# ssteinberg/wave_tracer

Measured on AMD Instinct MI355X. Metric: Msamples/sec (whole node), cornell-box 1440^2 wave-mode, higher is better.
Workload: dtype f32

## Files before the change

wave_tracer_amd/csrc/kernels_path.hip:

```cpp
#include "wtgpu_kernels.h"

namespace wtk {

__global__ void __launch_bounds__(kBlock) k_path_generate(launch_args_t a) {
    const uint32_t i = blockIdx.x * kBlock + threadIdx.x;
    if (i == 0) {
        uint32_t* ctl = a.st.ctl;
        ctl[CTL_COUNT0] = a.nb;
        ctl[CTL_COUNT1] = 0;
        ctl[CTL_BACK0] = ctl[CTL_BACK1] = 0;
        ctl[CTL_UTD_COUNT0] = ctl[CTL_UTD_COUNT1] = ctl[CTL_FSDQ_COUNT0] = ctl[CTL_FSDQ_COUNT1] = ctl[CTL_FSDQ_HEAD] = ctl[CTL_NEEQ_COUNT] = ctl[CTL_NEEQ_HEAD] = 0;
        ctl[CTL_HEAD_TRACE] = ctl[CTL_HEAD_INTERACT] = ctl[CTL_HEAVY_COUNT] = ctl[CTL_HEAVY_HEAD] = ctl[CTL_FSD_COUNTER] = ctl[CTL_ROUNDS] = 0;
        ctl[CTL_TPOL_COUNT0] = ctl[CTL_TPOL_COUNT1] = ctl[CTL_TPOL_HEAD] = ctl[CTL_TCONE_COUNT0] = ctl[CTL_TCONE_COUNT1] = ctl[CTL_TCONE_HEAD] = 0;
        ctl[CTL_INTB_COUNT] = ctl[CTL_INTB_HEAD] = ctl[CTL_GATHER_COUNT] = ctl[CTL_GATHER_HEAD] = ctl[CTL_INTC_COUNT] = ctl[CTL_INTC_HEAD] = 0;
        ctl[CTL_FTASK_COUNT] = ctl[CTL_FTASK_HEAD] = ctl[CTL_FSPLIT_HEAD] = ctl[CTL_EPOOL_COUNT] = ctl[CTL_FSD_ECOUNTER] = 0;
        ctl[CTL_INTD_COUNT] = ctl[CTL_INTD_HEAD] = 0;
    }
    if (i >= a.nb) return;
    const uint64_t j = a.j0 + i;
    const uint32_t pix = (uint32_t)(j % a.npix);
    const uint64_t s = a.sample_begin + j / a.npix;
    const uint64_t sample_id = ((uint64_t)pix << 32) | (s & 0xFFFFFFFFull);
    path_walk_t pw;
    path_generate(a.sc, a.seed, sample_id, pix % a.sc.sensor.width, pix / a.sc.sensor.width, pw);
    soa_store(a.st.walks, a.st.walk_words, i, pw);
}

#ifdef WTGPU_FSD_WATCH
// ... 241 lines not shown
```

wave_tracer_amd/csrc/kernels_trace.hip:

```cpp
#include "wtgpu_kernels.h"

namespace wtk {

}
#include "kernels_trace_refill.h"
namespace wtk {

__global__ void __launch_bounds__(kBlock, WTGPU_LB_TRACE) k_trace_refill(launch_args_t a, int in, int first_round, uint32_t round) { trace_refill_body(a, in, first_round, round); }

#ifndef WTGPU_SM_EXACT_MIN
#define WTGPU_SM_EXACT_MIN 24
#endif
#ifndef WTGPU_SM_SPLIT_NODE
#define WTGPU_SM_SPLIT_NODE 0
#endif
#ifndef WTGPU_SM_BOTH
#define WTGPU_SM_BOTH 0
#endif
enum : int { PH_IDLE = 0, PH_NODE = 1, PH_TRI = 2, PH_EXACT = 3, PH_SERVE = 4, PH_POLICY = 5, PH_RAYDONE = 6 };
#ifdef WTGPU_SM_PROF
#define SP_DECL() unsigned long long sp_t[8] = {0, 0, 0, 0, 0, 0, 0, 0}, sp_l[8] = {0, 0, 0, 0, 0, 0, 0, 0}, sp_n[8] = {0, 0, 0, 0, 0, 0, 0, 0}; long long sp_c = 0
#define SP_BEGIN() sp_c = clock64()
#define SP_END(i, mask) do { const long long d_ = clock64() - sp_c; sp_t[i] += (unsigned long long)d_; sp_l[i] += (unsigned long long)d_ * (unsigned long long)__popcll(mask); sp_n[i] += 1; } while (0)
#else
// ... 300 lines not shown
    for (;;) {
        const int need = aw_next(sc, env, rt, stack, aw, q, r);
        if (need != AW_TEST) return need == AW_QUERY;
        aw_test_done(aw, cone_attempt_too_short_by(sc, env, aw.cand, aw.sr, aw.min_df_prog));
    }
}
#ifndef WTGPU_LB_STAGE
#define WTGPU_LB_STAGE 3
#endif
__global__ void __launch_bounds__(kBlock, WTGPU_LB_STAGE) k_tr_axis(launch_args_t a, int in, int first_round, uint32_t round) {
    __shared__ stack_entry_t lds[kLdsStack * kBlock];
    uint32_t* ctl = a.st.ctl;
    const uint32_t n = queue_count(ctl, in);
    if (blockIdx.x == 0 && threadIdx.x == 0) {
        trace_round_begin(ctl, in, round, n);
        ctl[CTL_TCONE_HEAD] = 0;
        ctl[CTL_TPOL_COUNT1] = 0;
    }
    bdpt_counters_t ctr;
    memset(&ctr, 0, sizeof(ctr));
    stack_entry_t spill[kSpillStack];
    stack_ref_t stack;
    lds_stack(lds, spill, stack);
    const bool rt = a.sc.sensor.ray_trace_only || a.sc.opts.force_ray_tracing;
    const int lane = threadIdx.x & 63;
    uint32_t* stage = trace_stage_words(a);
    uint32_t* coneq = trace_cone_queue(a);
    for (;;) {
        const uint32_t base = wave_grab(ctl + CTL_HEAD_TRACE);
        if (base >= n) break;
        const uint32_t qi = base + (uint32_t)lane;
        bool fin = false, query = false;
        uint32_t w = 0;
        trav_result_t r;
        if (qi < n) {
            w = queue_walk(a, ctl, in, qi, first_round);
            const walk_trace_in_t wk = walk_load_trace_in(a.st.walks, a.st.walk_words, w);
            trace_stage_t ts;
            ts.env = walk_trace_envelope(a.sc, wk);
            ray_hit_t ah;
            const bool axis_hit = ads_intersect_ray(a.sc, ts.env.o, ts.env.d, range_t{0.f, WT_INF}, stack, ah);
            aw_begin(ts.aw, wavenum_to_wavelen_m(wk.k), WT_INF, axis_hit, ah, a.cone_budget, true, !(a.collect_list & 1u) || (a.collect_list & 2u), a.lane_cache ? wk.prev_offset_tuid : kInvalid);
            ts.aw.use_cache = a.lane_cache;
            query = tr_policy_run(a.sc, ts.env, rt, stack, ts.aw, r);
            fin = !query;
            if (query) soa_store(stage, kStageWords, w, ts);
        }
        wave_append(coneq, ctl + CTL_TCONE_COUNT0, query, w);
        tr_finish(a, ctl, ctr, fin, w, r);
    }
    if (a.count_stats) flush_counters(a.st.counters, ctr);
}
#ifndef WTGPU_CONE_REFILL_MIN
#define WTGPU_CONE_REFILL_MIN 16
#endif
#ifndef WTGPU_CONE_DEFER
#define WTGPU_CONE_DEFER 0
#endif
__global__ void __launch_bounds__(kBlock, WTGPU_LB_STAGE) k_tr_cone(launch_args_t a, uint32_t it) {
    __shared__ stack_entry_t lds[kLdsStack * kBlock];
#if WTGPU_CONE_DEFER
    __shared__ float lds_tri[12 * kBlock];
    float* my_tri = lds_tri + threadIdx.x;
    bool wait = false;
#endif
    uint32_t* ctl = a.st.ctl;
    const uint32_t n = ctl[CTL_TCONE_COUNT0 + (it & 1u)];
    if (blockIdx.x == 0 && threadIdx.x == 0) {
        ctl[CTL_TPOL_HEAD] = 0;
        ctl[CTL_TCONE_COUNT0 + ((it + 1u) & 1u)] = 0;
    }
    bdpt_counters_t ctr;
    memset(&ctr, 0, sizeof(ctr));
    stack_entry_t spill[kSpillStack];
    stack_ref_t stack;
    lds_stack(lds, spill, stack);
    const lane_nodes_t ns = lane_nodes(a.sc);
    const int lane = threadIdx.x & 63;
    const unsigned long long below = (1ull << lane) - 1ull;
    uint32_t* stage = trace_stage_words(a);
    const uint32_t* coneq = trace_cone_queue(a);
    uint32_t* polq = trace_pol_queue(a);
    uint32_t* pol_count = ctl + CTL_TPOL_COUNT0 + ((it + 1u) & 1u);
    int st = 0;
    uint32_t w = 0;
    cone_t env;
    cone_query_t q;
    memset(&env, 0, sizeof(env));
    memset(&q, 0, sizeof(q));
    bool exhausted = false;
    SP_DECL();
    for (;;) {
        uint32_t* slot = a.st.tris + (size_t)w * kTriListWords;
        const uint_list_t tris{slot, 1u, (a.collect_list & 1u) ? kMaxConeTris : 0u, reinterpret_cast<float*>(slot + kMaxConeTris)};
        bool fin = false, again = false;
        trav_result_t r;
        SP_BEGIN();
        const unsigned long long sp_m0 = __ballot(st == 2);
        (void)sp_m0;
        if (st == 2) {
            cq_end(env, tris, q);
            axis_walk_t aw;
            soa_load(stage + offsetof(trace_stage_t, aw) / 4, kStageWords, w, aw);
            fin = aw_query_done(a.sc, env, aw, q.rec, r);
            again = !fin;
            if (again) {
                stage[(size_t)w * kStageWords + (offsetof(trace_stage_t, aw) + offsetof(axis_walk_t, seg)) / 4] = aw.seg;
                stage[(size_t)w * kStageWords + (offsetof(trace_stage_t, aw) + offsetof(axis_walk_t, short_tuid)) / 4] = aw.short_tuid;
            }
            st = 0;
        }
        wave_append(polq, pol_count, again, w);
        tr_finish(a, ctl, ctr, fin, w, r);
        SP_END(0, sp_m0);
        {
            const unsigned long long im = __ballot(st == 0);
            const int n_run = __popcll(__ballot(st == 1));
            if (!exhausted && im && (__popcll(im) >= WTGPU_CONE_REFILL_MIN || n_run == 0)) {
                uint32_t base = 0;
                if (lane == 0) base = atomicAdd(ctl + CTL_TCONE_HEAD, (uint32_t)__popcll(im));
                base = (uint32_t)__shfl((int)base, 0, 64);
                if (base + (uint32_t)__popcll(im) >= n) exhausted = true;
                const uint32_t qi = base + (uint32_t)__popcll(im & below);
                SP_BEGIN();
                const unsigned long long sp_m1 = __ballot(st == 0 && qi < n);
                (void)sp_m1;
                if (st == 0 && qi < n) {
                    w = coneq[qi];
                    soa_load(stage, kStageWords, w, env);
                    const size_t o = (size_t)w * kStageWords + offsetof(trace_stage_t, aw) / 4;
                    const range_t sr{__uint_as_float(stage[o + offsetof(axis_walk_t, sr) / 4]), __uint_as_float(stage[o + offsetof(axis_walk_t, sr) / 4 + 1])};
                    const float min_df_prog = __uint_as_float(stage[o + offsetof(axis_walk_t, min_df_prog) / 4]);
                    cq_begin(a.sc, env, sr, kMajorAxisToZScale, stack, a.cone_budget, min_df_prog, q);
                    st = cq_running(q) ? 1 : 2;
                }
                SP_END(1, sp_m1);
            }
        }
        const int running = __popcll(__ballot(st == 1));
        if (running == 0) {
            if (__ballot(st == 2)) continue;
            if (exhausted) break;
            continue;
// ... 91 lines not shown
#endif
    }
    if (a.count_stats) flush_counters(a.st.counters, ctr);
#ifdef WTGPU_SM_PROF
    if (lane == 0)
        for (int i = 0; i < 8; ++i) {
            atomicAdd(a.st.counters + kNumCounters + 32 + i, sp_t[i]);
            atomicAdd(a.st.counters + kNumCounters + 40 + i, sp_l[i]);
            atomicAdd(a.st.counters + kNumCounters + 48 + i, sp_n[i]);
        }
#endif
}
__global__ void __launch_bounds__(kBlock, WTGPU_LB_STAGE) k_tr_policy(launch_args_t a, uint32_t it) {
    __shared__ stack_entry_t lds[kBlock];
    uint32_t* ctl = a.st.ctl;
    const uint32_t n = ctl[CTL_TPOL_COUNT0 + (it & 1u)];
    if (blockIdx.x == 0 && threadIdx.x == 0) {
        ctl[CTL_TCONE_HEAD] = 0;
        ctl[CTL_TPOL_COUNT0 + ((it + 1u) & 1u)] = 0;
    }
    bdpt_counters_t ctr;
    memset(&ctr, 0, sizeof(ctr));
    const stack_ref_t stack = make_stack_ref(lds + threadIdx.x, kBlock, 1, 1, nullptr);
    const bool rt = a.sc.sensor.ray_trace_only || a.sc.opts.force_ray_tracing;
    const int lane = threadIdx.x & 63;
    uint32_t* stage = trace_stage_words(a);
    const uint32_t* polq = trace_pol_queue(a);
    uint32_t* coneq = trace_cone_queue(a);
    for (;;) {
        const uint32_t base = wave_grab(ctl + CTL_TPOL_HEAD);
        if (base >= n) break;
        const uint32_t qi = base + (uint32_t)lane;
        bool fin = false, query = false;
        uint32_t w = 0;
        trav_result_t r;
        if (qi < n) {
            w = polq[qi];
            trace_stage_t ts;
            soa_load(stage, kStageWords, w, ts);
            query = tr_policy_run(a.sc, ts.env, rt, stack, ts.aw, r);
            fin = !query;
            if (query) soa_store(stage + offsetof(trace_stage_t, aw) / 4, kStageWords, w, ts.aw);
        }
        wave_append(coneq, ctl + CTL_TCONE_COUNT0 + (it & 1u), query, w);
        tr_finish(a, ctl, ctr, fin, w, r);
    }
    if (a.count_stats) flush_counters(a.st.counters, ctr);
}
__global__ void __launch_bounds__(kBlock, WTGPU_LB_TRACE) k_tr_tail(launch_args_t a, uint32_t it) {
    __shared__ stack_entry_t lds[kLdsStack * kBlock];
    uint32_t* ctl = a.st.ctl;
    const uint32_t n = ctl[CTL_TPOL_COUNT0 + (it & 1u)];
    if (blockIdx.x == 0 && threadIdx.x == 0) ctl[CTL_TCONE_COUNT0] = ctl[CTL_TCONE_COUNT1] = 0;
    bdpt_counters_t ctr;
    memset(&ctr, 0, sizeof(ctr));
    stack_entry_t spill[kSpillStack];
    stack_ref_t stack;
    lds_stack(lds, spill, stack);
    const lane_nodes_t ns = lane_nodes(a.sc);
    const bool rt = a.sc.sensor.ray_trace_only || a.sc.opts.force_ray_tracing;
    const int lane = threadIdx.x & 63;
    uint32_t* stage = trace_stage_words(a);
    const uint32_t* polq = trace_pol_queue(a);
    for (;;) {
        const uint32_t base = wave_grab(ctl + CTL_TPOL_HEAD);
        if (base >= n) break;
        const uint32_t qi = base + (uint32_t)lane;
        const bool have = qi < n;
        uint32_t w = 0;
        trav_result_t r;
        if (have) {
            w = polq[qi];
            trace_stage_t ts;
            soa_load(stage, kStageWords, w, ts);
            uint32_t* slot = a.st.tris + (size_t)w * kTriListWords;
            const uint_list_t tris{slot, 1u, (a.collect_list & 1u) ? kMaxConeTris : 0u, reinterpret_cast<float*>(slot + kMaxConeTris)};
            cone_query_t q;
            for (;;) {
                const int need = aw_next(a.sc, ts.env, rt, stack, ts.aw, q, r);
                if (need == AW_FINAL) break;
                if (need == AW_TEST) {
                    aw_test_done(ts.aw, cone_attempt_too_short_by(a.sc, ts.env, ts.aw.cand, ts.aw.sr, ts.aw.min_df_prog));
                    continue;
                }
                while (cq_running(q)) {
                    while (q.s > 0 && q.leaf == 0) cq_node_step(ns, ts.env, stack, q);
                    if (q.leaf != 0) cq_leaf_step(a.sc, ts.env, stack, tris, q);
// ... 161 lines not shown
```

wave_tracer_amd/csrc/kernels_walk.hip:

```cpp
#include "wtgpu_kernels.h"
#include "kernels_trace_refill.h"

namespace wtk {

__global__ void __launch_bounds__(kBlock) k_generate(launch_args_t a) {
    const uint32_t i = blockIdx.x * kBlock + threadIdx.x;
    if (i == 0) {
        uint32_t* ctl = a.st.ctl;
        ctl[CTL_COUNT0] = 2 * a.nb;
        ctl[CTL_COUNT1] = 0;
        ctl[CTL_BACK0] = ctl[CTL_BACK1] = 0;
        ctl[CTL_HEAD_TRACE] = ctl[CTL_HEAD_INTERACT] = ctl[CTL_HEAVY_COUNT] = ctl[CTL_HEAVY_HEAD] = ctl[CTL_FSD_COUNTER] = ctl[CTL_ROUNDS] = 0;
        ctl[CTL_TPOL_COUNT0] = ctl[CTL_TPOL_COUNT1] = ctl[CTL_TPOL_HEAD] = ctl[CTL_TCONE_COUNT0] = ctl[CTL_TCONE_COUNT1] = ctl[CTL_TCONE_HEAD] = 0;
        ctl[CTL_INTB_COUNT] = ctl[CTL_INTB_HEAD] = ctl[CTL_GATHER_COUNT] = ctl[CTL_GATHER_HEAD] = ctl[CTL_INTC_COUNT] = ctl[CTL_INTC_HEAD] = 0;
        ctl[CTL_FTASK_COUNT] = ctl[CTL_FTASK_HEAD] = ctl[CTL_FSPLIT_HEAD] = ctl[CTL_EPOOL_COUNT] = ctl[CTL_FSD_ECOUNTER] = 0;
        ctl[CTL_INTD_COUNT] = ctl[CTL_INTD_HEAD] = 0;
    }
    if (i >= a.nb) return;
    const uint64_t j = a.j0 + i;
    const uint32_t pix = (uint32_t)(j % a.npix);
    const uint64_t s = a.sample_begin + j / a.npix;
    const uint64_t sample_id = ((uint64_t)pix << 32) | (s & 0xFFFFFFFFull);
    const size_t W2 = 2 * (size_t)a.st.cap;
    sample_ctx_t ctx;
    walk_t sw, ew;
    const vertex_store_t svs{a.st.verts, a.st.vert_words, i}, evs{a.st.verts, a.st.vert_words, (size_t)a.st.cap + i};
    bdpt_generate(a.sc, a.seed, sample_id, pix % a.sc.sensor.width, pix / a.sc.sensor.width, ctx, sw, ew, svs, evs);
    soa_store(a.st.ctx, kCtxWords, i, ctx);
// ... 346 lines not shown
```

wave_tracer_amd/csrc/wtgpu.hip:

```cpp
#include <hip/hip_runtime.h>
#include <chrono>
#include <rccl/rccl.h>

#include <atomic>
#include <cmath>
#include <cstdio>
#include <cstdlib>
#include <algorithm>
#include <cstring>
#include <memory>
#include <mutex>
#include <thread>
#include <string>
#include <vector>

#include "wtgpu_kernels.h"
#include "wtgpu_test_hooks.h"
#include "scene_abi_check.h"
#include "host/scene_builder.h"

namespace {

thread_local std::string g_err;
int fail(int code, const std::string& msg) {
// ... 62 lines not shown
    std::atomic<int> paused{0};
    std::mutex capture_mutex;
    wtgpu_capture_cb capture_cb = nullptr;
    void* capture_user = nullptr;
    uint32_t* query_scratch = nullptr;
    size_t query_scratch_bytes = 0;
    double ab_ms[2] = {0, 0};
    uint64_t ab_mismatch = 0, ab_walks = 0, ab_rounds = 0;
    uint64_t light_rounds_run = 0;
    struct knobs_t {
        uint32_t cone_budget = 0, count_stats = 1, profile = 0, no_lists = 0, stagger_round = 0, lane_cache = 1, heavy_cache = 1, split_queues = 1;
        uint32_t shrink_r1 = 8, shrink_f1 = 4, shrink_r2 = 16, shrink_f2 = 32, shrink_h1 = 4, decay_q = 0, decay_c = 4;
        uint32_t heavy_waves_per_cu = 8, round_blocks_per_cu = 8, grid_div_b = 4, grid_div_c = 1, grid_div_hard = 4, grid_mul_flux = 2, coop_aperture_min = 8, heavy_probe = 1, flux_task_tris = kFluxTaskTris;
        uint32_t coop_io = 0, primary_axis = 0, sorted_interact = 0, staged_connect = 0, conn_pool = 16, grid_div_cls[4] = {1, 4, 2, 4};
        uint32_t trace_staged = 1, trace_stages = 3, trace_staged_rounds = 4;
        uint32_t trace_sm = 0, trace_ab = 0;
        uint32_t light_rounds = 1;
        uint32_t max_rounds = kWalkIterLimit;
        uint32_t first_rounds = 0, rounds_margin = 2, tiled_splat = 1;
        int dbg_stage = 1 << 30;
    } knobs;
};

struct wtgpu_comm {
    ncclComm_t comm = nullptr;
    int device = -1, world = 0, rank = 0;
};

struct device_guard_t {
    int prev = -1;
// ... 311 lines not shown
    k.stagger_round = std::min<uint32_t>(u("WTGPU_STAGGER_ROUND", 0), kMaxWalkIters - 1);
    k.profile = u("WTGPU_PROFILE", 0);
    k.no_lists = getenv("WTGPU_NO_LISTS") ? 1u : 0u;
    k.heavy_waves_per_cu = std::max(1u, u("WTGPU_HEAVY_WAVES", 8));
    k.round_blocks_per_cu = std::max(1u, u("WTGPU_ROUND_BLOCKS", 8));
    k.grid_div_b = std::max(1u, u("WTGPU_GRID_B", 4));
    k.grid_div_c = std::max(1u, u("WTGPU_GRID_C", 1));
    k.grid_div_hard = std::max(1u, u("WTGPU_GRID_HARD", 4));
    k.grid_mul_flux = std::max(1u, u("WTGPU_GRID_FLUX", 2));
    k.heavy_probe = u("WTGPU_HEAVY_PROBE", 1);
    k.trace_sm = u("WTGPU_TRACE_SM", k.trace_sm);
    k.trace_ab = u("WTGPU_TRACE_AB", 0);
    k.trace_staged = u("WTGPU_TRACE_STAGED", k.trace_staged);
    k.trace_staged_rounds = u("WTGPU_TRACE_STAGED_ROUNDS", k.trace_staged_rounds);
    k.trace_stages = std::min(16u, std::max(1u, u("WTGPU_TRACE_STAGES", k.trace_stages)));
    k.sorted_interact = u("WTGPU_SORTED_INTERACT", 0);
    k.primary_axis = u("WTGPU_PRIMARY_AXIS", 0);
    k.coop_io = u("WTGPU_COOP_IO", 0);
    k.staged_connect = u("WTGPU_STAGED_CONNECT", 0);
    k.conn_pool = std::max(1u, u("WTGPU_CONN_POOL", 16));
    if (const char* e = getenv("WTGPU_GRID_CLS")) {
        unsigned v[4] = {1, 4, 2, 4};
        sscanf(e, "%u,%u,%u,%u", &v[0], &v[1], &v[2], &v[3]);
        for (int c = 0; c < 4; ++c) k.grid_div_cls[c] = std::max(1u, v[c]);
    }
    k.flux_task_tris = std::max(64u, u("WTGPU_FLUX_TASK_TRIS", kFluxTaskTris));
    k.coop_aperture_min = u("WTGPU_COOP_APERTURE_MIN", 8);
    if (const char* e = getenv("WTGPU_DEBUG_STAGE")) k.dbg_stage = atoi(e);
    if (const char* e = getenv("WTGPU_TIMING")) s->timing = atoi(e) != 0;
}
// ... 93 lines not shown
    s->d_tri_class = nullptr;
    if (h.n_tris > 0 && h.opts.integrator == INTEGRATOR_BDPT) {
        std::vector<unsigned char> cls(h.n_tris);
        for (uint32_t t = 0; t < h.n_tris; ++t) cls[t] = (unsigned char)walk_class_of_triangle(h, t);
        if ((rc = upload(s, cls.data(), cls.size(), &s->d_tri_class)) != WTGPU_OK) return rc;
    }

    const uint64_t npix = (uint64_t)h.sensor.width * h.sensor.height;
    uint32_t n_slices = 3;
    if (const char* e = getenv("WTGPU_STREAMS")) n_slices = (uint32_t)std::max(1, atoi(e));
    uint64_t batch_cap = max_batch ? std::min<uint64_t>(max_batch, 1u << 24) : std::min<uint64_t>(npix, 1u << 22);
    n_slices = (uint32_t)std::min<uint64_t>(n_slices, std::max<uint64_t>(1, batch_cap / 64));
    {
        const bool pm = h.opts.integrator != INTEGRATOR_BDPT;
        const uint64_t mv = (uint64_t)h.opts.max_depth + 2;
        uint64_t per_sample = 4ull * (2 * ((pm ? kPathWalkWords : kWalkWords) + (pm ? 0 : mv * kVertexWords) + kTravWords + kStageWords + 2 + kTriListWords) + kCtxWords) + 64ull * 28ull + 2048ull;
        if (pm) per_sample += 2ull * 48ull * sizeof(utd_edge_rec_t) + sizeof(path_nee_rec_t) + 3ull * 4ull + 4ull + sizeof(uint2);
        else per_sample += (s->knobs.staged_connect ? (uint64_t)s->knobs.conn_pool * (sizeof(conn_pending_t) + 4ull) : 0ull) + (s->knobs.sorted_interact ? 4ull * 2ull * kNumWalkClasses : 0ull);
        uint64_t budget = 224ull << 30;
        if (const char* e = getenv("WTGPU_STATE_GB")) budget = (uint64_t)std::max(1, atoi(e)) << 30;
        size_t free_b = 0, total_b = 0;
        if (hipMemGetInfo(&free_b, &total_b) == hipSuccess && free_b > 0) budget = std::min<uint64_t>(budget, (uint64_t)((double)free_b * 0.85));
        const uint64_t fixed = (uint64_t)n_slices * ((1ull << 23) * 4ull + (1ull << 22) * 8ull + (64ull << 20));
        budget = budget > 2 * fixed ? budget - fixed : budget / 2;
        const uint64_t fit = std::max<uint64_t>(4096, budget / per_sample / n_slices);
        if (batch_cap > fit) batch_cap = fit;
    }
    unsigned long long* counters = nullptr;
    if ((rc = dmalloc(s, &counters, kNumCounters + kProfSlots + 1))) return rc;
    HIP_CHECK(hipMemset(counters, 0, (kNumCounters + kProfSlots + 1) * sizeof(unsigned long long)));
    s->slices.resize(n_slices);
// ... 43 lines not shown
            } else
                X.pend_cap = 0;
            s->pend_cap = X.pend_cap;
            s->n_chunks = X.n_chunks;
            bdpt_ext_t* dX = nullptr;
            if ((rc = dmalloc(s, &dX, 1))) return rc;
            HIP_CHECK(hipMemcpy(dX, &X, sizeof(X), hipMemcpyHostToDevice));
            st.ext = dX;
        }
        if ((rc = dmalloc(s, &st.verts, path_mode ? 1 : (size_t)st.max_verts * kVertexWords * W2))) return rc;
        if ((rc = dmalloc(s, &st.ctx, kCtxWords * (size_t)st.cap))) return rc;
        if ((rc = dmalloc(s, &st.trav, (kTravWords + kStageWords) * W2))) return rc;
        if ((rc = dmalloc(s, &st.tris, (size_t)kTriListWords * W2))) return rc;
        if ((rc = dmalloc(s, &st.queue[0], W2))) return rc;
        if ((rc = dmalloc(s, &st.queue[1], W2))) return rc;
        if ((rc = dmalloc(s, &st.heavy_queue, 3 * W2))) return rc;
        if ((rc = dmalloc(s, &st.intb_queue, W2))) return rc;
        if ((rc = dmalloc(s, &st.gather_queue, W2))) return rc;
        if ((rc = dmalloc(s, &st.intc_queue, W2))) return rc;
        if ((rc = dmalloc(s, &st.intd_queue, W2))) return rc;
        st.ftask_cap = path_mode ? 1u : (1u << 22);
        if ((rc = dmalloc(s, &st.ftasks, (size_t)st.ftask_cap))) return rc;
        if ((rc = dmalloc(s, &st.facc, path_mode ? 1 : W2))) return rc;
        st.epool_cap = 1u << 23;
        if ((rc = dmalloc(s, &st.epool, (size_t)st.epool_cap))) return rc;
        if ((rc = dmalloc(s, &st.ctl, (size_t)CTL_WORDS))) return rc;
        HIP_CHECK(hipMemset(st.ctl, 0, CTL_WORDS * sizeof(uint32_t)));
        st.fsd_cap = (h.opts.FSD && !h.opts.force_ray_tracing && !path_mode) ? (uint32_t)std::min<uint64_t>(W2, 1u << 22) : 1u;
        if ((rc = dmalloc(s, &st.fsd_hdr, st.fsd_cap))) return rc;
        st.fsd_ecap = st.fsd_cap > 1 ? (uint32_t)std::min<uint64_t>(64ull * st.cap + kFsdMaxEdges, 1ull << 28) : 1u;
        if ((rc = dmalloc(s, &st.fsd_edges, (size_t)st.fsd_ecap))) return rc;
        if ((rc = dmalloc(s, &st.strat_items, path_mode ? 1 : (size_t)kNumKeys * st.cap))) return rc;
        if ((rc = dmalloc(s, &st.strat_count, (size_t)kNumKeys))) return rc;
        if ((rc = dmalloc(s, &st.strat_prefix, (size_t)kNumKeys + 1))) return rc;
        if ((rc = dmalloc(s, &st.lacc, 4 * (size_t)st.cap))) return rc;
        HIP_CHECK(hipMemset(st.strat_count, 0, kNumKeys * sizeof(uint32_t)));
        HIP_CHECK(hipStreamCreateWithFlags(&s->streams[k], hipStreamNonBlocking));
        HIP_CHECK(hipEventCreateWithFlags(&s->ev_done[k], hipEventDisableTiming));
    }
    HIP_CHECK(hipEventCreateWithFlags(&s->ev_begin, hipEventDisableTiming));
    s->recs.resize(4 * (size_t)n_slices);
    s->pending.assign(n_slices, wtgpu_scene::pending_t{});
// ... 862 lines not shown
```

wave_tracer_amd/csrc/wtgpu_kernels.h:

```cpp
#pragma once
#include <hip/hip_runtime.h>

#include <cstddef>
#include <cstdint>
#include <cstring>

#include "../../include/wtgpu.h"
#include "wt/bdpt.h"
#include "wt/coop.h"
#include "wt/coop_fsd.h"
#include "wt/coop_utd.h"
#include "wt/path.h"

using namespace wt;

namespace wtk {


#ifndef WTGPU_LB_TRACE
#define WTGPU_LB_TRACE 3
#endif
#ifndef WTGPU_LB_HEAVY
#define WTGPU_LB_HEAVY 2
#endif
// ... 11 lines not shown
#endif
#ifndef WTGPU_LB_CONNECT
#define WTGPU_LB_CONNECT 2
#endif
constexpr uint32_t kFluxTaskTris = 2048;
constexpr int kBlock = 128;
#ifndef WTGPU_LDS_STACK
#define WTGPU_LDS_STACK 20
#endif
constexpr int kLdsStack = WTGPU_LDS_STACK;
constexpr uint32_t kConeBudget = 96;
constexpr int kSpillStack = 64 - kLdsStack;

enum : uint32_t { CTL_STRAT_HEAD_OPEN = 25, CTL_UTD_COUNT0 = 26, CTL_UTD_COUNT1 = 27, CTL_FSDQ_COUNT0 = 28, CTL_FSDQ_COUNT1 = 29, CTL_FSDQ_HEAD = 30, CTL_NEEQ_COUNT = 31, CTL_NEEQ_HEAD = 32, CTL_COUNT0 = 0, CTL_COUNT1 = 1, CTL_HEAD_TRACE = 2, CTL_HEAD_INTERACT = 3, CTL_HEAVY_COUNT = 4, CTL_HEAVY_HEAD = 5, CTL_FSD_COUNTER = 6,
                  CTL_ROUNDS = 7, CTL_STRAT_HEAD = 8, CTL_INTB_COUNT = 9, CTL_INTB_HEAD = 10, CTL_GATHER_COUNT = 11, CTL_GATHER_HEAD = 12, CTL_INTC_COUNT = 13, CTL_INTC_HEAD = 14, CTL_FTASK_COUNT = 15, CTL_FTASK_HEAD = 16, CTL_FSPLIT_HEAD = 17, CTL_EPOOL_COUNT = 18, CTL_FSD_ECOUNTER = 19, CTL_INTD_COUNT = 20, CTL_INTD_HEAD = 21, CTL_BACK0 = 22, CTL_BACK1 = 23,
                  CTL_TPOL_COUNT0 = 41, CTL_TPOL_COUNT1 = 42, CTL_TPOL_HEAD = 43, CTL_TCONE_COUNT0 = 44, CTL_TCONE_COUNT1 = 45, CTL_TCONE_HEAD = 46,
                  CTL_CLS_COUNT0 = 33, CTL_CLS_HEAD0 = 37,
                  CTL_LIGHT_DONE = 47, CTL_LIGHT_STOP = 48,
                  CTL_WORDS = 56 };
constexpr uint32_t kTriListWords = 128;
constexpr uint32_t kGatherMarker = 0xFFFFFFFEu;
constexpr uint32_t kApertureMarker = 0xFFFFFFFDu, kNullApertureMarker = 0xFFFFFFFCu;
__host__ __device__ inline bool is_region_marker(uint32_t t) { return t == kGatherMarker || t == kApertureMarker; }
constexpr uint32_t kKeyDim = kMaxVerts + 2, kNumKeys = kKeyDim * kKeyDim;

struct device_state_t {
    uint64_t cap = 0;
    uint32_t max_verts = 0;
    uint32_t walk_words = 0;
    size_t vert_words = 0;
    uint32_t* walks = nullptr;
    uint32_t* verts = nullptr;
    uint32_t* ctx = nullptr;
    uint32_t* trav = nullptr;
// ... 68 lines not shown
    uint32_t nb;
    uint32_t npix;
    uint64_t sample_begin;
    uint32_t count_stats;
    uint32_t cone_budget;
    uint32_t flux_task_tris;
    uint32_t heavy_probe;
    uint32_t coop_aperture_min;
    uint32_t profile;
    uint32_t split_queues;
    uint32_t lane_cache, heavy_cache;
    uint32_t collect_list;
};

WT_D uint32_t* trace_stage_words(const launch_args_t& a) { return a.st.trav + kTravWords * 2 * (size_t)a.st.cap; }
WT_D uint32_t* trace_pol_queue(const launch_args_t& a) { return a.st.heavy_queue + 2 * (size_t)a.st.cap; }
WT_D uint32_t* trace_cone_queue(const launch_args_t& a) { return a.st.heavy_queue + 4 * (size_t)a.st.cap; }
WT_D void lds_stack(stack_entry_t* lds, stack_entry_t* spill, stack_ref_t& s, uint32_t block = kBlock) {
    s = make_stack_ref(lds + threadIdx.x, block, kLdsStack + kSpillStack, kLdsStack, spill);
}

WT_D void flush_counters(unsigned long long* g, const bdpt_counters_t& c) {
    const unsigned long long* p = reinterpret_cast<const unsigned long long*>(&c);
#pragma unroll
    for (size_t i = 0; i < kNumCounters; ++i) {
        unsigned long long v = p[i];
        for (int off = 32; off > 0; off >>= 1) v += __shfl_down(v, off, 64);
        if ((threadIdx.x & 63) == 0 && v) atomicAdd(&g[i], v);
    }
}

WT_D void walk_ident(const launch_args_t& a, uint32_t w, uint32_t& i, uint32_t& stream) {
// ... 35 lines not shown
    base = (uint32_t)__shfl((int)base, leader, 64);
    if (pred) queue[base + (uint32_t)__popcll(m & ((1ull << lane) - 1ull))] = w;
}

WT_D void queue_append(const launch_args_t& a, uint32_t* ctl, int out, bool pred, uint32_t w) {
    const bool back = pred && w >= a.st.cap && a.split_queues;
    wave_append(a.st.queue[out], ctl + CTL_COUNT0 + out, pred && !back, w);
    const unsigned long long m = __ballot(back);
    if (!m) return;
    const int lane = threadIdx.x & 63;
    const int leader = __ffsll((long long)m) - 1;
    uint32_t base = 0;
    if (lane == leader) base = atomicAdd(ctl + CTL_BACK0 + out, (uint32_t)__popcll(m));
    base = (uint32_t)__shfl((int)base, leader, 64);
    if (back) a.st.queue[out][2 * (size_t)a.st.cap - 1 - (base + (uint32_t)__popcll(m & ((1ull << lane) - 1ull)))] = w;
}

constexpr int kIoRows = 32;
template <int W>
constexpr int io_pitch() { return (W & 1) ? W : W + 1; }
template <int W, class T>
WT_D void wave_load_records(const uint32_t* base, size_t stride, uint32_t idx, bool valid, uint32_t* lds, T& out) {
    static_assert(sizeof(T) == 4 * W, "record size");
    constexpr int P = io_pitch<W>();
    const int lane = threadIdx.x & 63;
    uint32_t* o = reinterpret_cast<uint32_t*>(&out);
    const unsigned long long all = __ballot(valid);
#pragma unroll 1
    for (int h = 0; h < 2; ++h) {
        unsigned long long m = all & (h ? 0xFFFFFFFF00000000ull : 0x00000000FFFFFFFFull);
// ... 104 lines not shown
```

Before: 30.66.

## Replace trace cone/policy queues with binned multi-queue supporting spatial/XCD keys

Swaps the single flat cone and policy work queues for a binned queue structure. Each bin has its own count and head counter plus an overflow segment. Producers pick a bin from a Morton code of the hit point or from the XCD id, and consumers start at their home bin and then steal from the others. The aim is better spatial coherence and less atomic contention across XCDs. With the default knobs (queue_bins=1) it acts as a single bin but adds extra ballot/readlane overhead and per-block resets.

Measured after the change: 30.69, median of 4. Within noise of the previous version (+0.1%).

```diff
diff --git a/wave_tracer_amd/csrc/kernels_path.hip b/wave_tracer_amd/csrc/kernels_path.hip
--- a/wave_tracer_amd/csrc/kernels_path.hip
+++ b/wave_tracer_amd/csrc/kernels_path.hip
@@ -11,7 +11,7 @@
         ctl[CTL_BACK0] = ctl[CTL_BACK1] = 0;
         ctl[CTL_UTD_COUNT0] = ctl[CTL_UTD_COUNT1] = ctl[CTL_FSDQ_COUNT0] = ctl[CTL_FSDQ_COUNT1] = ctl[CTL_FSDQ_HEAD] = ctl[CTL_NEEQ_COUNT] = ctl[CTL_NEEQ_HEAD] = 0;
         ctl[CTL_HEAD_TRACE] = ctl[CTL_HEAD_INTERACT] = ctl[CTL_HEAVY_COUNT] = ctl[CTL_HEAVY_HEAD] = ctl[CTL_FSD_COUNTER] = ctl[CTL_ROUNDS] = 0;
-        ctl[CTL_TPOL_COUNT0] = ctl[CTL_TPOL_COUNT1] = ctl[CTL_TPOL_HEAD] = ctl[CTL_TCONE_COUNT0] = ctl[CTL_TCONE_COUNT1] = ctl[CTL_TCONE_HEAD] = 0;
+        for (uint32_t k = CTL_TCONE_COUNT0; k < CTL_BINQ_END; ++k) ctl[k] = 0;
         ctl[CTL_INTB_COUNT] = ctl[CTL_INTB_HEAD] = ctl[CTL_GATHER_COUNT] = ctl[CTL_GATHER_HEAD] = ctl[CTL_INTC_COUNT] = ctl[CTL_INTC_HEAD] = 0;
         ctl[CTL_FTASK_COUNT] = ctl[CTL_FTASK_HEAD] = ctl[CTL_FSPLIT_HEAD] = ctl[CTL_EPOOL_COUNT] = ctl[CTL_FSD_ECOUNTER] = 0;
         ctl[CTL_INTD_COUNT] = ctl[CTL_INTD_HEAD] = 0;
diff --git a/wave_tracer_amd/csrc/kernels_trace.hip b/wave_tracer_amd/csrc/kernels_trace.hip
--- a/wave_tracer_amd/csrc/kernels_trace.hip
+++ b/wave_tracer_amd/csrc/kernels_trace.hip
@@ -338,9 +338,9 @@
     const uint32_t n = queue_count(ctl, in);
     if (blockIdx.x == 0 && threadIdx.x == 0) {
         trace_round_begin(ctl, in, round, n);
-        ctl[CTL_TCONE_HEAD] = 0;
-        ctl[CTL_TPOL_COUNT1] = 0;
-    }
+    }
+    binq_reset(ctl + CTL_TCONE_HEAD);
+    binq_reset(ctl + CTL_TPOL_COUNT0 + kBinSlots);
     bdpt_counters_t ctr;
     memset(&ctr, 0, sizeof(ctr));
     stack_entry_t spill[kSpillStack];
@@ -349,13 +349,13 @@
     const bool rt = a.sc.sensor.ray_trace_only || a.sc.opts.force_ray_tracing;
     const int lane = threadIdx.x & 63;
     uint32_t* stage = trace_stage_words(a);
-    uint32_t* coneq = trace_cone_queue(a);
+    const binq_t coneq = trace_cone_binq(a, 0);
     for (;;) {
         const uint32_t base = wave_grab(ctl + CTL_HEAD_TRACE);
         if (base >= n) break;
         const uint32_t qi = base + (uint32_t)lane;
         bool fin = false, query = false;
-        uint32_t w = 0;
+        uint32_t w = 0, bin = 0;
         trav_result_t r;
         if (qi < n) {
             w = queue_walk(a, ctl, in, qi, first_round);
@@ -368,9 +368,12 @@
             ts.aw.use_cache = a.lane_cache;
             query = tr_policy_run(a.sc, ts.env, rt, stack, ts.aw, r);
             fin = !query;
-            if (query) soa_store(stage, kStageWords, w, ts);
-        }
-        wave_append(coneq, ctl + CTL_TCONE_COUNT0, query, w);
+            if (query) {
+                soa_store(stage, kStageWords, w, ts);
+                bin = trace_bin(a.sc, coneq, ts.env, ts.aw);
+            }
+        }
+        binq_append(coneq, query, w, bin);
         tr_finish(a, ctl, ctr, fin, w, r);
     }
     if (a.count_stats) flush_counters(a.st.counters, ctr);
@@ -389,11 +392,9 @@
     bool wait = false;
 #endif
     uint32_t* ctl = a.st.ctl;
-    const uint32_t n = ctl[CTL_TCONE_COUNT0 + (it & 1u)];
-    if (blockIdx.x == 0 && threadIdx.x == 0) {
-        ctl[CTL_TPOL_HEAD] = 0;
-        ctl[CTL_TCONE_COUNT0 + ((it + 1u) & 1u)] = 0;
-    }
+    const binq_t coneq = binq_consumer(trace_cone_binq(a, it & 1u));
+    binq_reset(ctl + CTL_TPOL_HEAD);
+    binq_reset(ctl + CTL_TCONE_COUNT0 + kBinSlots * ((it + 1u) & 1u));
     bdpt_counters_t ctr;
     memset(&ctr, 0, sizeof(ctr));
     stack_entry_t spill[kSpillStack];
@@ -403,9 +404,9 @@
     const int lane = threadIdx.x & 63;
     const unsigned long long below = (1ull << lane) - 1ull;
     uint32_t* stage = trace_stage_words(a);
-    const uint32_t* coneq = trace_cone_queue(a);
-    uint32_t* polq = trace_pol_queue(a);
-    uint32_t* pol_count = ctl + CTL_TPOL_COUNT0 + ((it + 1u) & 1u);
+    const binq_t polq = trace_pol_binq(a, (it + 1u) & 1u);
+    const uint32_t home = binq_home(coneq);
+    uint32_t vis = 0;
     int st = 0;
     uint32_t w = 0;
     cone_t env;
@@ -418,6 +419,7 @@
         uint32_t* slot = a.st.tris + (size_t)w * kTriListWords;
         const uint_list_t tris{slot, 1u, (a.collect_list & 1u) ? kMaxConeTris : 0u, reinterpret_cast<float*>(slot + kMaxConeTris)};
         bool fin = false, again = false;
+        uint32_t bin = 0;
         trav_result_t r;
         SP_BEGIN();
         const unsigned long long sp_m0 = __ballot(st == 2);
@@ -431,26 +433,26 @@
             if (again) {
                 stage[(size_t)w * kStageWords + (offsetof(trace_stage_t, aw) + offsetof(axis_walk_t, seg)) / 4] = aw.seg;
                 stage[(size_t)w * kStageWords + (offsetof(trace_stage_t, aw) + offsetof(axis_walk_t, short_tuid)) / 4] = aw.short_tuid;
+                bin = trace_bin(a.sc, polq, env, aw);
             }
             st = 0;
         }
-        wave_append(polq, pol_count, again, w);
+        binq_append(polq, again, w, bin);
         tr_finish(a, ctl, ctr, fin, w, r);
         SP_END(0, sp_m0);
         {
             const unsigned long long im = __ballot(st == 0);
             const int n_run = __popcll(__ballot(st == 1));
             if (!exhausted && im && (__popcll(im) >= WTGPU_CONE_REFILL_MIN || n_run == 0)) {
-                uint32_t base = 0;
-                if (lane == 0) base = atomicAdd(ctl + CTL_TCONE_HEAD, (uint32_t)__popcll(im));
-                base = (uint32_t)__shfl((int)base, 0, 64);
-                if (base + (uint32_t)__popcll(im) >= n) exhausted = true;
+                uint32_t base = 0, n = 0;
+                size_t off = 0;
+                if (!binq_grab(coneq, home, vis, (uint32_t)__popcll(im), base, n, off) || vis > coneq.nbins) exhausted = true;
                 const uint32_t qi = base + (uint32_t)__popcll(im & below);
                 SP_BEGIN();
                 const unsigned long long sp_m1 = __ballot(st == 0 && qi < n);
                 (void)sp_m1;
                 if (st == 0 && qi < n) {
-                    w = coneq[qi];
+                    w = coneq.data[off + qi];
                     soa_load(stage, kStageWords, w, env);
                     const size_t o = (size_t)w * kStageWords + offsetof(trace_stage_t, aw) / 4;
                     const range_t sr{__uint_as_float(stage[o + offsetof(axis_walk_t, sr) / 4]), __uint_as_float(stage[o + offsetof(axis_walk_t, sr) / 4 + 1])};
@@ -572,35 +574,38 @@
 __global__ void __launch_bounds__(kBlock, WTGPU_LB_STAGE) k_tr_policy(launch_args_t a, uint32_t it) {
     __shared__ stack_entry_t lds[kBlock];
     uint32_t* ctl = a.st.ctl;
-    const uint32_t n = ctl[CTL_TPOL_COUNT0 + (it & 1u)];
-    if (blockIdx.x == 0 && threadIdx.x == 0) {
-        ctl[CTL_TCONE_HEAD] = 0;
-        ctl[CTL_TPOL_COUNT0 + ((it + 1u) & 1u)] = 0;
-    }
+    const binq_t polq = binq_consumer(trace_pol_binq(a, it & 1u));
+    binq_reset(ctl + CTL_TCONE_HEAD);
+    binq_reset(ctl + CTL_TPOL_COUNT0 + kBinSlots * ((it + 1u) & 1u));
     bdpt_counters_t ctr;
     memset(&ctr, 0, sizeof(ctr));
     const stack_ref_t stack = make_stack_ref(lds + threadIdx.x, kBlock, 1, 1, nullptr);
     const bool rt = a.sc.sensor.ray_trace_only || a.sc.opts.force_ray_tracing;
     const int lane = threadIdx.x & 63;
     uint32_t* stage = trace_stage_words(a);
-    const uint32_t* polq = trace_pol_queue(a);
-    uint32_t* coneq = trace_cone_queue(a);
+    const binq_t coneq = trace_cone_binq(a, it & 1u);
+    const uint32_t home = binq_home(polq);
+    uint32_t vis = 0;
     for (;;) {
-        const uint32_t base = wave_grab(ctl + CTL_TPOL_HEAD);
-        if (base >= n) break;
+        uint32_t base = 0, n = 0;
+        size_t off = 0;
+        if (!binq_grab(polq, home, vis, 64u, base, n, off)) break;
         const uint32_t qi = base + (uint32_t)lane;
         bool fin = false, query = false;
-        uint32_t w = 0;
+        uint32_t w = 0, bin = 0;
         trav_result_t r;
         if (qi < n) {
-            w = polq[qi];
+            w = polq.data[off + qi];
             trace_stage_t ts;
             soa_load(stage, kStageWords, w, ts);
             query = tr_policy_run(a.sc, ts.env, rt, stack, ts.aw, r);
             fin = !query;
-            if (query) soa_store(stage + offsetof(trace_stage_t, aw) / 4, kStageWords, w, ts.aw);
-        }
-        wave_append(coneq, ctl + CTL_TCONE_COUNT0 + (it & 1u), query, w);
+            if (query) {
+                soa_store(stage + offsetof(trace_stage_t, aw) / 4, kStageWords, w, ts.aw);
+                bin = trace_bin(a.sc, coneq, ts.env, ts.aw);
+            }
+        }
+        binq_append(coneq, query, w, bin);
         tr_finish(a, ctl, ctr, fin, w, r);
     }
     if (a.count_stats) flush_counters(a.st.counters, ctr);
@@ -608,8 +613,9 @@
 __global__ void __launch_bounds__(kBlock, WTGPU_LB_TRACE) k_tr_tail(launch_args_t a, uint32_t it) {
     __shared__ stack_entry_t lds[kLdsStack * kBlock];
     uint32_t* ctl = a.st.ctl;
-    const uint32_t n = ctl[CTL_TPOL_COUNT0 + (it & 1u)];
-    if (blockIdx.x == 0 && threadIdx.x == 0) ctl[CTL_TCONE_COUNT0] = ctl[CTL_TCONE_COUNT1] = 0;
+    const binq_t polq = binq_consumer(trace_pol_binq(a, it & 1u));
+    binq_reset(ctl + CTL_TCONE_COUNT0);
+    binq_reset(ctl + CTL_TCONE_COUNT0 + kBinSlots);
     bdpt_counters_t ctr;
     memset(&ctr, 0, sizeof(ctr));
     stack_entry_t spill[kSpillStack];
@@ -619,16 +625,18 @@
     const bool rt = a.sc.sensor.ray_trace_only || a.sc.opts.force_ray_tracing;
     const int lane = threadIdx.x & 63;
     uint32_t* stage = trace_stage_words(a);
-    const uint32_t* polq = trace_pol_queue(a);
+    const uint32_t home = binq_home(polq);
+    uint32_t vis = 0;
     for (;;) {
-        const uint32_t base = wave_grab(ctl + CTL_TPOL_HEAD);
-        if (base >= n) break;
+        uint32_t base = 0, n = 0;
+        size_t off = 0;
+        if (!binq_grab(polq, home, vis, 64u, base, n, off)) break;
         const uint32_t qi = base + (uint32_t)lane;
         const bool have = qi < n;
         uint32_t w = 0;
         trav_result_t r;
         if (have) {
-            w = polq[qi];
+            w = polq.data[off + qi];
             trace_stage_t ts;
             soa_load(stage, kStageWords, w, ts);
             uint32_t* slot = a.st.tris + (size_t)w * kTriListWords;
diff --git a/wave_tracer_amd/csrc/kernels_walk.hip b/wave_tracer_amd/csrc/kernels_walk.hip
--- a/wave_tracer_amd/csrc/kernels_walk.hip
+++ b/wave_tracer_amd/csrc/kernels_walk.hip
@@ -11,7 +11,7 @@
         ctl[CTL_COUNT1] = 0;
         ctl[CTL_BACK0] = ctl[CTL_BACK1] = 0;
         ctl[CTL_HEAD_TRACE] = ctl[CTL_HEAD_INTERACT] = ctl[CTL_HEAVY_COUNT] = ctl[CTL_HEAVY_HEAD] = ctl[CTL_FSD_COUNTER] = ctl[CTL_ROUNDS] = 0;
-        ctl[CTL_TPOL_COUNT0] = ctl[CTL_TPOL_COUNT1] = ctl[CTL_TPOL_HEAD] = ctl[CTL_TCONE_COUNT0] = ctl[CTL_TCONE_COUNT1] = ctl[CTL_TCONE_HEAD] = 0;
+        for (uint32_t k = CTL_TCONE_COUNT0; k < CTL_BINQ_END; ++k) ctl[k] = 0;
         ctl[CTL_INTB_COUNT] = ctl[CTL_INTB_HEAD] = ctl[CTL_GATHER_COUNT] = ctl[CTL_GATHER_HEAD] = ctl[CTL_INTC_COUNT] = ctl[CTL_INTC_HEAD] = 0;
         ctl[CTL_FTASK_COUNT] = ctl[CTL_FTASK_HEAD] = ctl[CTL_FSPLIT_HEAD] = ctl[CTL_EPOOL_COUNT] = ctl[CTL_FSD_ECOUNTER] = 0;
         ctl[CTL_INTD_COUNT] = ctl[CTL_INTD_HEAD] = 0;
diff --git a/wave_tracer_amd/csrc/wtgpu.hip b/wave_tracer_amd/csrc/wtgpu.hip
--- a/wave_tracer_amd/csrc/wtgpu.hip
+++ b/wave_tracer_amd/csrc/wtgpu.hip
@@ -100,6 +100,7 @@
         uint32_t heavy_waves_per_cu = 8, round_blocks_per_cu = 8, grid_div_b = 4, grid_div_c = 1, grid_div_hard = 4, grid_mul_flux = 2, coop_aperture_min = 8, heavy_probe = 1, flux_task_tris = kFluxTaskTris;
         uint32_t coop_io = 0, primary_axis = 0, sorted_interact = 0, staged_connect = 0, conn_pool = 16, grid_div_cls[4] = {1, 4, 2, 4};
         uint32_t trace_staged = 1, trace_stages = 3, trace_staged_rounds = 4;
+        uint32_t queue_bins = 1, queue_bin_seg = 0, queue_key = 1;
         uint32_t trace_sm = 0, trace_ab = 0;
         uint32_t light_rounds = 1;
         uint32_t max_rounds = kWalkIterLimit;
@@ -441,6 +442,9 @@
     k.trace_staged = u("WTGPU_TRACE_STAGED", k.trace_staged);
     k.trace_staged_rounds = u("WTGPU_TRACE_STAGED_ROUNDS", k.trace_staged_rounds);
     k.trace_stages = std::min(16u, std::max(1u, u("WTGPU_TRACE_STAGES", k.trace_stages)));
+    k.queue_bins = std::min(kMaxQueueBins, std::max(1u, u("WTGPU_QUEUE_BINS", k.queue_bins)));
+    k.queue_bin_seg = u("WTGPU_QUEUE_BIN_SEG", 0);
+    k.queue_key = u("WTGPU_QUEUE_KEY", 1) ? 1u : 0u;
     k.sorted_interact = u("WTGPU_SORTED_INTERACT", 0);
     k.primary_axis = u("WTGPU_PRIMARY_AXIS", 0);
     k.coop_io = u("WTGPU_COOP_IO", 0);
@@ -564,7 +568,7 @@
     {
         const bool pm = h.opts.integrator != INTEGRATOR_BDPT;
         const uint64_t mv = (uint64_t)h.opts.max_depth + 2;
-        uint64_t per_sample = 4ull * (2 * ((pm ? kPathWalkWords : kWalkWords) + (pm ? 0 : mv * kVertexWords) + kTravWords + kStageWords + 2 + kTriListWords) + kCtxWords) + 64ull * 28ull + 2048ull;
+        uint64_t per_sample = 4ull * (2 * ((pm ? kPathWalkWords : kWalkWords) + (pm ? 0 : mv * kVertexWords) + kTravWords + kStageWords + 4 + kTriListWords) + kCtxWords) + 64ull * 28ull + 2048ull;
         if (pm) per_sample += 2ull * 48ull * sizeof(utd_edge_rec_t) + sizeof(path_nee_rec_t) + 3ull * 4ull + 4ull + sizeof(uint2);
         else per_sample += (s->knobs.staged_connect ? (uint64_t)s->knobs.conn_pool * (sizeof(conn_pending_t) + 4ull) : 0ull) + (s->knobs.sorted_interact ? 4ull * 2ull * kNumWalkClasses : 0ull);
         uint64_t budget = 224ull << 30;
@@ -638,7 +642,7 @@
         if ((rc = dmalloc(s, &st.tris, (size_t)kTriListWords * W2))) return rc;
         if ((rc = dmalloc(s, &st.queue[0], W2))) return rc;
         if ((rc = dmalloc(s, &st.queue[1], W2))) return rc;
-        if ((rc = dmalloc(s, &st.heavy_queue, 3 * W2))) return rc;
+        if ((rc = dmalloc(s, &st.heavy_queue, W2 + 2 * binq_words(W2)))) return rc;
         if ((rc = dmalloc(s, &st.intb_queue, W2))) return rc;
         if ((rc = dmalloc(s, &st.gather_queue, W2))) return rc;
         if ((rc = dmalloc(s, &st.intc_queue, W2))) return rc;
@@ -650,6 +654,12 @@
         if ((rc = dmalloc(s, &st.epool, (size_t)st.epool_cap))) return rc;
         if ((rc = dmalloc(s, &st.ctl, (size_t)CTL_WORDS))) return rc;
         HIP_CHECK(hipMemset(st.ctl, 0, CTL_WORDS * sizeof(uint32_t)));
+        {
+            const uint32_t nbins = s->knobs.queue_bins, full = (uint32_t)((W2 + nbins - 1) / nbins);
+            const uint32_t shape[2] = {nbins, s->knobs.queue_bin_seg ? std::min(full, s->knobs.queue_bin_seg) : full};
+            HIP_CHECK(hipMemcpy(st.ctl + CTL_QBINS, shape, sizeof(shape), hipMemcpyHostToDevice));
+            HIP_CHECK(hipMemcpy(st.ctl + CTL_QKEY, &s->knobs.queue_key, 4, hipMemcpyHostToDevice));
+        }
         st.fsd_cap = (h.opts.FSD && !h.opts.force_ray_tracing && !path_mode) ? (uint32_t)std::min<uint64_t>(W2, 1u << 22) : 1u;
         if ((rc = dmalloc(s, &st.fsd_hdr, st.fsd_cap))) return rc;
         st.fsd_ecap = st.fsd_cap > 1 ? (uint32_t)std::min<uint64_t>(64ull * st.cap + kFsdMaxEdges, 1ull << 28) : 1u;
diff --git a/wave_tracer_amd/csrc/wtgpu_kernels.h b/wave_tracer_amd/csrc/wtgpu_kernels.h
--- a/wave_tracer_amd/csrc/wtgpu_kernels.h
+++ b/wave_tracer_amd/csrc/wtgpu_kernels.h
@@ -49,10 +49,10 @@
 
 enum : uint32_t { CTL_STRAT_HEAD_OPEN = 25, CTL_UTD_COUNT0 = 26, CTL_UTD_COUNT1 = 27, CTL_FSDQ_COUNT0 = 28, CTL_FSDQ_COUNT1 = 29, CTL_FSDQ_HEAD = 30, CTL_NEEQ_COUNT = 31, CTL_NEEQ_HEAD = 32, CTL_COUNT0 = 0, CTL_COUNT1 = 1, CTL_HEAD_TRACE = 2, CTL_HEAD_INTERACT = 3, CTL_HEAVY_COUNT = 4, CTL_HEAVY_HEAD = 5, CTL_FSD_COUNTER = 6,
                   CTL_ROUNDS = 7, CTL_STRAT_HEAD = 8, CTL_INTB_COUNT = 9, CTL_INTB_HEAD = 10, CTL_GATHER_COUNT = 11, CTL_GATHER_HEAD = 12, CTL_INTC_COUNT = 13, CTL_INTC_HEAD = 14, CTL_FTASK_COUNT = 15, CTL_FTASK_HEAD = 16, CTL_FSPLIT_HEAD = 17, CTL_EPOOL_COUNT = 18, CTL_FSD_ECOUNTER = 19, CTL_INTD_COUNT = 20, CTL_INTD_HEAD = 21, CTL_BACK0 = 22, CTL_BACK1 = 23,
-                  CTL_TPOL_COUNT0 = 41, CTL_TPOL_COUNT1 = 42, CTL_TPOL_HEAD = 43, CTL_TCONE_COUNT0 = 44, CTL_TCONE_COUNT1 = 45, CTL_TCONE_HEAD = 46,
                   CTL_CLS_COUNT0 = 33, CTL_CLS_HEAD0 = 37,
                   CTL_LIGHT_DONE = 47, CTL_LIGHT_STOP = 48,
-                  CTL_WORDS = 56 };
+                  CTL_QBINS = 56, CTL_QSEG = 57, CTL_QKEY = 41, CTL_TCONE_COUNT0 = 58, CTL_TCONE_HEAD = 76, CTL_TPOL_COUNT0 = 85, CTL_TPOL_HEAD = 103, CTL_BINQ_END = 112,
+                  CTL_WORDS = 112 };
 constexpr uint32_t kTriListWords = 128;
 constexpr uint32_t kGatherMarker = 0xFFFFFFFEu;
 constexpr uint32_t kApertureMarker = 0xFFFFFFFDu, kNullApertureMarker = 0xFFFFFFFCu;
@@ -151,8 +151,57 @@
 };
 
 WT_D uint32_t* trace_stage_words(const launch_args_t& a) { return a.st.trav + kTravWords * 2 * (size_t)a.st.cap; }
+
+constexpr uint32_t kMaxQueueBins = 8, kBinSlots = kMaxQueueBins + 1;
+__host__ __device__ constexpr size_t binq_words(size_t cap) { return 2 * cap + kMaxQueueBins; }
+struct binq_t {
+    uint32_t* data;
+    uint32_t* count;
+    uint32_t* head;
+    uint32_t nbins, seg;
+    uint32_t key;
+    uint32_t sizes;
+};
 WT_D uint32_t* trace_pol_queue(const launch_args_t& a) { return a.st.heavy_queue + 2 * (size_t)a.st.cap; }
-WT_D uint32_t* trace_cone_queue(const launch_args_t& a) { return a.st.heavy_queue + 4 * (size_t)a.st.cap; }
+WT_D uint32_t* trace_cone_queue(const launch_args_t& a) { return trace_pol_queue(a) + binq_words(2 * (size_t)a.st.cap); }
+WT_D binq_t trace_pol_binq(const launch_args_t& a, uint32_t p) {
+    return binq_t{trace_pol_queue(a), a.st.ctl + CTL_TPOL_COUNT0 + kBinSlots * p, a.st.ctl + CTL_TPOL_HEAD, a.st.ctl[CTL_QBINS], a.st.ctl[CTL_QSEG], a.st.ctl[CTL_QKEY], 0u};
+}
+WT_D binq_t trace_cone_binq(const launch_args_t& a, uint32_t p) {
+    return binq_t{trace_cone_queue(a), a.st.ctl + CTL_TCONE_COUNT0 + kBinSlots * p, a.st.ctl + CTL_TCONE_HEAD, a.st.ctl[CTL_QBINS], a.st.ctl[CTL_QSEG], a.st.ctl[CTL_QKEY], 0u};
+}
+WT_D void binq_reset(uint32_t* words) {
+    if (blockIdx.x == 0 && threadIdx.x < kBinSlots) words[threadIdx.x] = 0;
+}
+WT_D uint32_t morton_spread10(uint32_t v) {
+    v &= 0x3FFu;
+    v = (v | (v << 16)) & 0x030000FFu;
+    v = (v | (v << 8)) & 0x0300F00Fu;
+    v = (v | (v << 4)) & 0x030C30C3u;
+    v = (v | (v << 2)) & 0x09249249u;
+    return v;
+}
+WT_D uint32_t bin_of_point(const scene_t& sc, const vec3& p, uint32_t nbins) {
+    auto cell = [](float x, float lo, float hi) {
+        const float t = (x - lo) / fmaxf(hi - lo, 1e-30f) * 1024.f;
+        return (uint32_t)fminf(fmaxf(t, 0.f), 1023.f);
+    };
+    const uint32_t code = (morton_spread10(cell(p.x, sc.world_min.x, sc.world_max.x)) << 2) | (morton_spread10(cell(p.y, sc.world_min.y, sc.world_max.y)) << 1) |
+                          morton_spread10(cell(p.z, sc.world_min.z, sc.world_max.z));
+    return (uint32_t)(((uint64_t)code * nbins) >> 30);
+}
+WT_D uint32_t xcd_id() {
+    uint32_t v;
+    asm volatile("s_getreg_b32 %0, hwreg(HW_REG_XCC_ID)" : "=s"(v));
+    return v & 0xFu;
+}
+WT_D uint32_t binq_home(const binq_t& q) { return xcd_id() % q.nbins; }
+WT_D uint32_t trace_bin(const scene_t& sc, const binq_t& q, const cone_t& env, const axis_walk_t& aw) {
+    if (q.nbins <= 1) return 0;
+    if (!q.key) return binq_home(q);
+    const vec3 p = aw.axis_hit ? env.o + env.d * aw.ah.dist : env.o;
+    return bin_of_point(sc, p, q.nbins);
+}
 WT_D void lds_stack(stack_entry_t* lds, stack_entry_t* spill, stack_ref_t& s, uint32_t block = kBlock) {
     s = make_stack_ref(lds + threadIdx.x, block, kLdsStack + kSpillStack, kLdsStack, spill);
 }
@@ -218,6 +267,64 @@
     if (lane == leader) base = atomicAdd(ctl + CTL_BACK0 + out, (uint32_t)__popcll(m));
     base = (uint32_t)__shfl((int)base, leader, 64);
     if (back) a.st.queue[out][2 * (size_t)a.st.cap - 1 - (base + (uint32_t)__popcll(m & ((1ull << lane) - 1ull)))] = w;
+}
+
+WT_D void binq_append(const binq_t& q, bool pred, uint32_t w, uint32_t bin) {
+    unsigned long long todo = __ballot(pred);
+    if (!todo) return;
+    const int lane = threadIdx.x & 63;
+    const unsigned long long below = (1ull << lane) - 1ull;
+    unsigned long long group = 0;
+    while (todo) {
+        const int leader = __ffsll((long long)todo) - 1;
+        const uint32_t b = (uint32_t)__builtin_amdgcn_readlane((int)bin, leader);
+        const bool mine = pred && bin == b;
+        const unsigned long long m = __ballot(mine);
+        todo &= ~m;
+        if (mine) group = m;
+    }
+    uint32_t base = 0;
+    if (pred && (group & below) == 0) base = atomicAdd(q.count + bin, (uint32_t)__popcll(group));
+    base = (uint32_t)__shfl((int)base, pred ? __ffsll((long long)group) - 1 : lane, 64);
+    const uint32_t k = base + (uint32_t)__popcll(group & below);
+    bool over = false;
+    if (pred) {
+        if (k < q.seg)
+            q.data[(size_t)bin * q.seg + k] = w;
+        else
+            over = true;
+    }
+    const unsigned long long mo = __ballot(over);
+    if (!mo) return;
+    const int leader = __ffsll((long long)mo) - 1;
+    uint32_t obase = 0;
+    if (lane == leader) obase = atomicAdd(q.count + kMaxQueueBins, (uint32_t)__popcll(mo));
+    obase = (uint32_t)__shfl((int)obase, leader, 64);
+    if (over) q.data[(size_t)q.nbins * q.seg + obase + (uint32_t)__popcll(mo & below)] = w;
+}
+WT_D binq_t binq_consumer(binq_t q) {
+    const uint32_t l = threadIdx.x & 63;
+    q.sizes = l < kMaxQueueBins ? min(q.count[l], q.seg) : (l == kMaxQueueBins ? q.count[kMaxQueueBins] : 0u);
+    return q;
+}
+WT_D uint32_t binq_size(const binq_t& q, uint32_t slot) { return (uint32_t)__builtin_amdgcn_readlane((int)q.sizes, (int)slot); }
+WT_D size_t binq_offset(const binq_t& q, uint32_t slot) { return (size_t)(slot < kMaxQueueBins ? slot : q.nbins) * q.seg; }
+WT_D bool binq_grab(const binq_t& q, uint32_t home, uint32_t& vis, uint32_t inc, uint32_t& base, uint32_t& end, size_t& off) {
+    while (vis <= q.nbins) {
+        const uint32_t slot = vis < q.nbins ? (home + vis) % q.nbins : kMaxQueueBins;
+        const uint32_t size = binq_size(q, slot);
+        if (size > 0) {
+            base = wave_grab0(q.head + slot, inc);
+            if (base < size) {
+                end = size;
+                off = binq_offset(q, slot);
+                if (base + inc >= size) ++vis;
+                return true;
+            }
+        }
+        ++vis;
+    }
+    return false;
 }
 
 constexpr int kIoRows = 32;
```
